# VainF/Diff-Pruning

Measured on NVIDIA H100. Metric: taylor_score_unet_fwd_bwd_passes_per_sec, higher is better.
Workload: dtype f32

## Files before the change

### diff-pruning_b200/csrc/conv_tc.cu

```cuda
#include <cuda.h>
#include <cuda_fp16.h>
#include "common.cuh"
#include "sm90.cuh"
#include "sm90_host.cuh"

namespace {
using namespace sm90;

constexpr int BM = 128, BK = 64;
constexpr int A_BYTES = BM * 32 * 4;

struct TcParams {
  int Nimg, H, W;
  int Nout;
  int kchunks;
  int bw, bh, bn, tiles_w, tiles_h;
  float* y; long long ldy;
  const float* bias;
  const float* rowadd; long long ld_rowadd;
  const float* residual; long long ld_res;
  int accumulate;
  int vec4;
  int ntaps;
  signed char dh[9], dw[9], wt[9];
  int os, oa, ob, Ho, Wo;
  int in_stride;
  float alpha;
  int b_from_img;
  const uint32_t* amax_a;
  const uint32_t* amax_b;
  uint32_t* amax_out;
  int ksplit, it_per_split;
  float* ws; long long ws_split_stride; int ws_ld;
  const float* gx; long long gldx;
  int gH, gW, gC, gQ, gPQ, gS, gstride, gpad_t, gpad_l, gM;
  int relu;
};

__device__ __forceinline__ int amax_exponent(const uint32_t* slot) {
  const int E = (int)((__ldg(slot) >> 23) & 0xFFu);
  return min(max(E, 14), 254);
}
__device__ __forceinline__ float scale_up(int E) { return __uint_as_float((uint32_t)(267 - E) << 23); }
__device__ __forceinline__ float scale_dn(int E) { return __uint_as_float((uint32_t)(E - 13) << 23); }
constexpr float LO_SCALE = 2048.f, LO_UNSCALE = 1.f / 2048.f;
__device__ __forceinline__ void split2(float a, float b, uint32_t& h, uint32_t& l) {
  const __half2 hh = __floats2half2_rn(a, b);
  const float2 hf = __half22float2(hh);
  const __half2 ll = __floats2half2_rn((a - hf.x) * LO_SCALE, (b - hf.y) * LO_SCALE);
  h = *reinterpret_cast<const uint32_t*>(&hh);
  l = *reinterpret_cast<const uint32_t*>(&ll);
}
__device__ __forceinline__ void split1(float v, __half& h, __half& l) {
  h = __float2half_rn(v);
  l = __float2half_rn((v - __half2float(h)) * LO_SCALE);
}

constexpr int PS_STAGES = 3, PS_BN = 128;
constexpr int PS_B_BYTES = PS_BN * BK * 2;
constexpr int PS_STAGE_BYTES = 2 * A_BYTES + 2 * PS_B_BYTES;

template <bool ANY>
__global__ void __launch_bounds__(THREADS, 1)
conv_tc_ps_kernel(const __grid_constant__ CUtensorMap mapA, const __grid_constant__ CUtensorMap mapBh,
                  const __grid_constant__ CUtensorMap mapBl, const TcParams p, const int tiles_m, const int total_tiles) {
  const int total_work = total_tiles * p.ksplit;
  extern __shared__ uint8_t smem_raw[];
  const uint32_t raw = smem_u32(smem_raw);
  const uint32_t pad_to = ((raw + 1023u) & ~1023u) - raw;
  uint8_t* smem = smem_raw + pad_to;
  const uint32_t sbase = raw + pad_to;
  const uint32_t bar0 = sbase + PS_STAGES * PS_STAGE_BYTES;
  auto full_bar = [&](int s) { return bar0 + 8u * s; };
  auto empty_bar = [&](int s) { return bar0 + 8u * (PS_STAGES + s); };
  const int wg = threadIdx.x >> 7, tid = threadIdx.x & 127;
  if (threadIdx.x == 0) {
    for (int s = 0; s < PS_STAGES; ++s) { mbar_init(full_bar(s), ANY ? 1 + 128 : 1); mbar_init(empty_bar(s), 8); }
    mbar_init_fence();
  }
  __syncthreads();
  const int iters_per_tile = p.ntaps * p.kchunks;

  auto tile_coords = [&](int tile, int& q0, int& p0, int& n0, int& nblk) {
    nblk = tile / tiles_m;
    const int tile_m = tile - nblk * tiles_m;
    const int tw = tile_m % p.tiles_w;
    const int th = (tile_m / p.tiles_w) % p.tiles_h;
    const int tn = tile_m / (p.tiles_w * p.tiles_h);
    q0 = tw * p.bw; p0 = th * p.bh; n0 = tn * p.bn;
  };

  if (wg == 0) {
    setmaxnreg_dec<40>();
    if constexpr (ANY) {
      const int t = threadIdx.x;
      if (t == 0) { prefetch_map(&mapBh); prefetch_map(&mapBl); }
      const uint32_t sw = (uint32_t)(t & 7);
      uint32_t g = 0;
      for (int wi = blockIdx.x; wi < total_work; wi += gridDim.x) {
        const int tile = wi % total_tiles, it0 = (wi / total_tiles) * p.it_per_split, it1 = min(iters_per_tile, it0 + p.it_per_split);
        const int nblk = tile / tiles_m, m = (tile - nblk * tiles_m) * BM + t;
        const bool mv = m < p.gM;
        const int n = mv ? m / p.gPQ : 0, rem = m - n * p.gPQ, pq = rem / p.gQ;
        const int hb = pq * p.gstride - p.gpad_t, wb = (rem - pq * p.gQ) * p.gstride - p.gpad_l;
        const float* xn = p.gx + (long long)n * p.gH * p.gW * p.gldx;
        for (int it = it0; it < it1; ++it, ++g) {
          const int s = g % PS_STAGES;
          const uint32_t ph = (g / PS_STAGES) & 1u;
          mbar_wait(empty_bar(s), ph ^ 1u);
          const int tap = it / p.kchunks, kc = it - tap * p.kchunks;
          const int r = tap / p.gS, h = hb + r, w = wb + (tap - r * p.gS);
          const uint32_t st = sbase + s * PS_STAGE_BYTES;
          if (t == 0) {
            mbar_expect_tx(full_bar(s), 2 * PS_B_BYTES);
            tma_load_3d(st + 2 * A_BYTES, &mapBh, full_bar(s), kc * BK, nblk * PS_BN, tap);
            tma_load_3d(st + 2 * A_BYTES + PS_B_BYTES, &mapBl, full_bar(s), kc * BK, nblk * PS_BN, tap);
          }
          const bool v = mv && h >= 0 && h < p.gH && w >= 0 && w < p.gW;
          const int cleft = v ? p.gC - kc * BK : 0;
          const float* src = v ? xn + ((long long)h * p.gW + w) * p.gldx + kc * BK : p.gx;
#pragma unroll
          for (int j = 0; j < 16; ++j) {
            const int nb = min(max(cleft - 4 * j, 0), 4) * 4;
            cp_async16(st + (j >> 3) * A_BYTES + t * 128 + ((((uint32_t)j & 7u) ^ sw) << 4), nb ? src + 4 * j : p.gx, (uint32_t)nb);
          }
          cp_async_mbar_arrive(full_bar(s));
        }
      }
      return;
    }
    if (threadIdx.x == 0) {
      prefetch_map(&mapA); prefetch_map(&mapBh); prefetch_map(&mapBl);
      uint32_t g = 0;
      for (int wi = blockIdx.x; wi < total_work; wi += gridDim.x) {
        const int tile = wi % total_tiles, it0 = (wi / total_tiles) * p.it_per_split, it1 = min(iters_per_tile, it0 + p.it_per_split);
        int q0, p0, n0, nblk;
        tile_coords(tile, q0, p0, n0, nblk);
        for (int it = it0; it < it1; ++it, ++g) {
          const int s = g % PS_STAGES;
          const uint32_t ph = (g / PS_STAGES) & 1u;
          mbar_wait(empty_bar(s), ph ^ 1u);
          mbar_expect_tx(full_bar(s), PS_STAGE_BYTES);
          const int tap = it / p.kchunks, kc = it - tap * p.kchunks;
          const uint32_t st = sbase + s * PS_STAGE_BYTES;
          const int aw = q0 * p.in_stride + p.dw[tap], ah = p0 * p.in_stride + p.dh[tap];
          tma_load_4d(st, &mapA, full_bar(s), kc * BK, aw, ah, n0);
          tma_load_4d(st + A_BYTES, &mapA, full_bar(s), kc * BK + 32, aw, ah, n0);
          const int tapb = p.b_from_img ? n0 : p.wt[tap];
          tma_load_3d(st + 2 * A_BYTES, &mapBh, full_bar(s), kc * BK, nblk * PS_BN, tapb);
          tma_load_3d(st + 2 * A_BYTES + PS_B_BYTES, &mapBl, full_bar(s), kc * BK, nblk * PS_BN, tapb);
        }
      }
    }
    return;
  }
  setmaxnreg_inc<232>();
  const int c = wg - 1;
  const int warp = tid >> 5, lane = tid & 31;
  const uint32_t frag_row = (uint32_t)(64 * c + 16 * warp + (lane >> 2)) * 128 + 8 * (lane & 1);
  const uint32_t fsw = (uint32_t)(lane >> 2), fj = (uint32_t)((lane & 3) >> 1);
  const float sa = scale_up(amax_exponent(p.amax_a));
  const float f1 = scale_dn(amax_exponent(p.amax_a)), f2 = scale_dn(amax_exponent(p.amax_b)) * p.alpha;
  auto fin = [&](float main, float corr) { return fmaf(corr, LO_UNSCALE, main) * f1 * f2; };
  float amax = 0.f;
  uint32_t g = 0;
  for (int wi = blockIdx.x; wi < total_work; wi += gridDim.x) {
    const int tile = wi % total_tiles, it0 = (wi / total_tiles) * p.it_per_split, it1 = min(iters_per_tile, it0 + p.it_per_split);
    float acc[64], cor[64];
    uint32_t fh[2][4], fl[2][4];
    int prev_s = 0;
    for (int it = it0; it < it1; ++it, ++g) {
      const int s = g % PS_STAGES;
      const uint32_t ph = (g / PS_STAGES) & 1u;
      mbar_wait(full_bar(s), ph);
      const uint8_t* stp = smem + s * PS_STAGE_BYTES + frag_row;
      const uint32_t bst = sbase + s * PS_STAGE_BYTES + 2 * A_BYTES;
#pragma unroll
      for (int k = 0; k < BK / 16; ++k) {
        uint32_t (&ah)[4] = fh[k & 1];
        uint32_t (&al)[4] = fl[k & 1];
        const uint8_t* a = stp + (k >> 1) * A_BYTES;
        const uint32_t pos = ((4u * (k & 1) + fj) ^ fsw) << 4;
        const float2 v0 = *reinterpret_cast<const float2*>(a + pos), v1 = *reinterpret_cast<const float2*>(a + 1024 + pos);
        const float2 v2 = *reinterpret_cast<const float2*>(a + (pos ^ 32u)), v3 = *reinterpret_cast<const float2*>(a + 1024 + (pos ^ 32u));
        split2(v0.x * sa, v0.y * sa, ah[0], al[0]);
        split2(v1.x * sa, v1.y * sa, ah[1], al[1]);
        split2(v2.x * sa, v2.y * sa, ah[2], al[2]);
        split2(v3.x * sa, v3.y * sa, ah[3], al[3]);
        const uint64_t b_hi = desc_k(bst + k * 32), b_lo = desc_k(bst + PS_B_BYTES + k * 32);
        const uint32_t first = (it > it0 || k > 0) ? 1u : 0u;
        wgmma_fence();
        wgmma_f16_n128_rs<0>(acc, ah, b_hi, first);
        wgmma_f16_n128_rs<0>(cor, ah, b_lo, first);
        wgmma_f16_n128_rs<0>(cor, al, b_hi, 1u);
        wgmma_commit();
        wgmma_wait<1>();
        if (k == 0 && it > it0 && lane == 0) mbar_arrive(empty_bar(prev_s));
      }
      prev_s = s;
    }
    wgmma_wait<0>();
    fence_regs(acc); fence_regs(cor);
    if (lane == 0) mbar_arrive(empty_bar(prev_s));

    int q0, p0, n0, nblk;
    tile_coords(tile, q0, p0, n0, nblk);
#pragma unroll
    for (int i = 0; i < 2; ++i) {
      const int row = 64 * c + 16 * warp + (lane >> 2) + 8 * i;
      const int cb = 2 * (lane & 3);
      if (p.ksplit > 1) {
        float* wrow = p.ws + (long long)(wi / total_tiles) * p.ws_split_stride + ((long long)(tile - nblk * tiles_m) * BM + row) * p.ws_ld + nblk * PS_BN;
#pragma unroll
        for (int j = 0; j < 16; ++j)
          *reinterpret_cast<float2*>(wrow + 8 * j + cb) =
              make_float2(fin(acc[4 * j + 2 * i], cor[4 * j + 2 * i]), fin(acc[4 * j + 2 * i + 1], cor[4 * j + 2 * i + 1]));
        continue;
      }
      const int w_l = row % p.bw, h_l = (row / p.bw) % p.bh, n_l = row / (p.bw * p.bh);
      const int img = n0 + n_l;
      if (img >= p.Nimg) continue;
      if constexpr (ANY) { if (q0 + w_l >= p.Wo) continue; }
      const long long m = ((long long)img * p.Ho + ((p0 + h_l) * p.os + p.oa)) * p.Wo + ((q0 + w_l) * p.os + p.ob);
      float* yrow = p.y + m * p.ldy;
      const float* rrow = p.residual ? p.residual + m * p.ld_res : nullptr;
      const float* arow2 = p.rowadd ? p.rowadd + (long long)img * p.ld_rowadd : nullptr;
#pragma unroll
      for (int j = 0; j < 16; ++j) {
        const int col = nblk * PS_BN + 8 * j + cb;
        float o[2] = {fin(acc[4 * j + 2 * i], cor[4 * j + 2 * i]), fin(acc[4 * j + 2 * i + 1], cor[4 * j + 2 * i + 1])};
        if (p.vec4 && col + 2 <= p.Nout) {
          if (p.bias) { const float2 t = __ldg(reinterpret_cast<const float2*>(p.bias + col)); o[0] += t.x; o[1] += t.y; }
          if (arow2) { const float2 t = __ldg(reinterpret_cast<const float2*>(arow2 + col)); o[0] += t.x; o[1] += t.y; }
          if (rrow) { const float2 t = __ldg(reinterpret_cast<const float2*>(rrow + col)); o[0] += t.x; o[1] += t.y; }
          float2* dst = reinterpret_cast<float2*>(yrow + col);
          if (p.accumulate) { const float2 t = *dst; o[0] += t.x; o[1] += t.y; }
          if constexpr (ANY) { if (p.relu) { o[0] = fmaxf(o[0], 0.f); o[1] = fmaxf(o[1], 0.f); } }
          *dst = make_float2(o[0], o[1]);
          amax = fmaxf(amax, fmaxf(fabsf(o[0]), fabsf(o[1])));
        } else {
#pragma unroll
          for (int e = 0; e < 2; ++e) {
            const int cc = col + e;
            if (cc < p.Nout) {
              float ov = o[e];
              if (p.bias) ov += __ldg(p.bias + cc);
              if (arow2) ov += __ldg(arow2 + cc);
              if (rrow) ov += __ldg(rrow + cc);
              if (p.accumulate) ov += yrow[cc];
              if constexpr (ANY) { if (p.relu) ov = fmaxf(ov, 0.f); }
              yrow[cc] = ov;
              amax = fmaxf(amax, fabsf(ov));
            }
          }
        }
      }
    }
  }
  if (p.amax_out && p.ksplit == 1) amax_commit(p.amax_out, amax);
}

__global__ void __launch_bounds__(256) splitk_epilogue_kernel(const TcParams p, const int tiles_m) {
  const int c4 = (p.Nout + 3) >> 2;
  const long long total = (long long)tiles_m * BM * c4;
  float amax = 0.f;
  for (long long i = blockIdx.x * 256ll + threadIdx.x; i < total; i += (long long)gridDim.x * 256) {
    const long long grow = i / c4;
    const int c = (int)(i - grow * c4) << 2;
    const int tile_m = (int)(grow / BM), row = (int)(grow - (long long)tile_m * BM);
    const int tw = tile_m % p.tiles_w, th = (tile_m / p.tiles_w) % p.tiles_h, tn = tile_m / (p.tiles_w * p.tiles_h);
    const int w_l = row % p.bw, h_l = (row / p.bw) % p.bh, n_l = row / (p.bw * p.bh);
    const int img = tn * p.bn + n_l;
    if (img >= p.Nimg) continue;
    const float* src = p.ws + grow * p.ws_ld + c;
    float4 acc = *reinterpret_cast<const float4*>(src);
    for (int ks = 1; ks < p.ksplit; ++ks) {
      const float4 t = *reinterpret_cast<const float4*>(src + ks * p.ws_split_stride);
      acc.x += t.x; acc.y += t.y; acc.z += t.z; acc.w += t.w;
    }
    float o[4] = {acc.x, acc.y, acc.z, acc.w};
    const long long m = ((long long)img * p.Ho + ((th * p.bh + h_l) * p.os + p.oa)) * p.Wo + ((tw * p.bw + w_l) * p.os + p.ob);
    float* yrow = p.y + m * p.ldy;
#pragma unroll
    for (int e = 0; e < 4; ++e) {
      const int cc = c + e;
      if (cc < p.Nout) {
        float v = o[e];
        if (p.bias) v += __ldg(p.bias + cc);
        if (p.rowadd) v += __ldg(p.rowadd + (long long)img * p.ld_rowadd + cc);
        if (p.residual) v += __ldg(p.residual + m * p.ld_res + cc);
        if (p.accumulate) v += yrow[cc];
        yrow[cc] = v;
        amax = fmaxf(amax, fabsf(v));
      }
    }
  }
  if (p.amax_out) amax_commit(p.amax_out, amax);
}

__global__ void __launch_bounds__(256) splitk_flat_epilogue_kernel(const TcParams p) {
  const int c4 = (p.Nout + 3) >> 2;
  const long long total = (long long)p.gM * c4;
  float amax = 0.f;
  for (long long i = blockIdx.x * 256ll + threadIdx.x; i < total; i += (long long)gridDim.x * 256) {
    const long long m = i / c4;
    const int c = (int)(i - m * c4) << 2;
    const float* src = p.ws + m * p.ws_ld + c;
    float4 acc = *reinterpret_cast<const float4*>(src);
    for (int ks = 1; ks < p.ksplit; ++ks) {
      const float4 t = *reinterpret_cast<const float4*>(src + ks * p.ws_split_stride);
      acc.x += t.x; acc.y += t.y; acc.z += t.z; acc.w += t.w;
    }
    const float o[4] = {acc.x, acc.y, acc.z, acc.w};
    float* yrow = p.y + m * p.ldy;
#pragma unroll
    for (int e = 0; e < 4; ++e) {
      const int cc = c + e;
      if (cc < p.Nout) {
        float v = o[e];
        if (p.bias) v += __ldg(p.bias + cc);
        if (p.residual) v += __ldg(p.residual + m * p.ld_res + cc);
        if (p.accumulate) v += yrow[cc];
        if (p.relu) v = fmaxf(v, 0.f);
        yrow[cc] = v;
        amax = fmaxf(amax, fabsf(v));
      }
    }
  }
  if (p.amax_out) amax_commit(p.amax_out, amax);
}

struct WgParams {
  int Nimg, H, W, C, K;
  int R, S, pad;
  int bw, bh, bn, tiles_w, tiles_h;
  int total_chunks, chunks_per_split;
  int c_tiles;
  float* ws;
  int in_stride;
  const uint32_t* amax_x; const uint32_t* amax_y;
  float* bias_ws;
};
constexpr int WG_KPIX = 64;
constexpr int WG_BLK = WG_KPIX * 128;
constexpr int WG_STAGES = 3, WG_STAGE_BYTES = 8 * WG_BLK;

__global__ void __launch_bounds__(THREADS, 1)
wgrad_tc_kernel(const __grid_constant__ CUtensorMap mapDy, const __grid_constant__ CUtensorMap mapX, const WgParams p) {
  extern __shared__ uint8_t smem_raw[];
  const uint32_t raw = smem_u32(smem_raw);
  const uint32_t pad_to = ((raw + 1023u) & ~1023u) - raw;
  uint8_t* smem = smem_raw + pad_to;
  const uint32_t sbase = raw + pad_to;
  const uint32_t bar0 = sbase + WG_STAGES * WG_STAGE_BYTES;
  auto full_bar = [&](int s) { return bar0 + 8u * s; };
  auto empty_bar = [&](int s) { return bar0 + 8u * (WG_STAGES + s); };
  const int wg = threadIdx.x >> 7, tid = threadIdx.x & 127;
  if (threadIdx.x == 0) {
    for (int s = 0; s < WG_STAGES; ++s) { mbar_init(full_bar(s), 1); mbar_init(empty_bar(s), 8); }
    mbar_init_fence();
  }
  __syncthreads();

  const int T = p.R * p.S;
  int tile = blockIdx.x;
  const int tap = tile % T; tile /= T;
  const int ct = tile % p.c_tiles;
  const int kt = tile / p.c_tiles;
  const int r = tap / p.S, sx = tap - r * p.S;
  const int chunk0 = blockIdx.y * p.chunks_per_split;
  const int chunk1 = min(p.total_chunks, chunk0 + p.chunks_per_split);
  const int num_iters = max(0, chunk1 - chunk0);
  const int dy_boxes = min(4, (p.K - kt * 128 + 31) >> 5), x_boxes = min(4, (p.C - ct * 128 + 31) >> 5);

  if (wg == 0) {
    setmaxnreg_dec<24>();
    if (threadIdx.x == 0) {
      prefetch_map(&mapDy); prefetch_map(&mapX);
      for (int it = 0; it < num_iters; ++it) {
        const int s = it % WG_STAGES;
        const uint32_t ph = (uint32_t)(it / WG_STAGES) & 1u;
        mbar_wait(empty_bar(s), ph ^ 1u);
        mbar_expect_tx(full_bar(s), (uint32_t)((dy_boxes + x_boxes) * WG_BLK));
        const int chunk = chunk0 + it;
        const int tw = chunk % p.tiles_w;
        const int th = (chunk / p.tiles_w) % p.tiles_h;
        const int tn = chunk / (p.tiles_w * p.tiles_h);
        const int q0 = tw * p.bw, p0 = th * p.bh, n0 = tn * p.bn;
        const uint32_t st = sbase + s * WG_STAGE_BYTES;
        const int xw = q0 * p.in_stride + sx - p.pad, xh = p0 * p.in_stride + r - p.pad;
#pragma unroll
        for (int b = 0; b < 4; ++b) {
          const uint32_t slot = (uint32_t)((b & 1) * 2 + (b >> 1));
          if (b < dy_boxes) tma_load_4d(st + slot * WG_BLK, &mapDy, full_bar(s), kt * 128 + b * 32, q0, p0, n0);
          if (b < x_boxes) tma_load_4d(st + (4 + slot) * WG_BLK, &mapX, full_bar(s), ct * 128 + b * 32, xw, xh, n0);
        }
      }
    }
    return;
  }
  setmaxnreg_inc<240>();
  const int c = wg - 1;
  const int warp = tid >> 5, lane = tid & 31;
  const int Ey = amax_exponent(p.amax_y), Ex = amax_exponent(p.amax_x);
  const float sy = scale_up(Ey), sxs = scale_up(Ex);
  const bool dy_valid = 2 * c + (warp >> 1) < dy_boxes;
  const uint32_t cb = (uint32_t)(16 * (warp & 1) + (lane >> 2)), pe = (uint32_t)(2 * (lane & 3));
  const uint32_t dy_off = (uint32_t)((warp >> 1) * 2 + c) * WG_BLK + pe * 128 + (((cb >> 2) ^ pe) << 4) + (cb & 3) * 4;
  const int xp = tid & 63, xh = tid >> 6;
  const bool x_valid = 2 * c + xh < x_boxes;
  const uint32_t xsw = (uint32_t)(xp & 7);
  float bsum[2] = {0.f, 0.f};
  float acc[64], cor[64];
  int prev_s = 0;
  auto stage = [&](uint32_t (&fah)[4][4], uint32_t (&fal)[4][4], const int it) {
    const int s = it % WG_STAGES;
    const uint32_t ph = (uint32_t)(it / WG_STAGES) & 1u;
    mbar_wait(full_bar(s), ph);
    uint8_t* stp = smem + s * WG_STAGE_BYTES;
    uint8_t* x0 = stp + 4 * WG_BLK + c * WG_BLK + xp * 128;
    uint8_t* x1 = x0 + 2 * WG_BLK;
    float4 xv[8];
    if (x_valid) {
      const uint8_t* src = xh ? x1 : x0;
#pragma unroll
      for (int j = 0; j < 8; ++j) xv[j] = *reinterpret_cast<const float4*>(src + ((j ^ xsw) << 4));
    }
    named_sync(1 + c, 128);
    if (x_valid) {
#pragma unroll
      for (int m = 0; m < 4; ++m) {
        const float4 u0 = xv[2 * m], u1 = xv[2 * m + 1];
        uint4 hq, lq;
        split2(u0.x * sxs, u0.y * sxs, hq.x, lq.x);
        split2(u0.z * sxs, u0.w * sxs, hq.y, lq.y);
        split2(u1.x * sxs, u1.y * sxs, hq.z, lq.z);
        split2(u1.z * sxs, u1.w * sxs, hq.w, lq.w);
        const uint32_t pos = (uint32_t)(((4 * xh + m) ^ xsw) << 4);
        *reinterpret_cast<uint4*>(x0 + pos) = hq;
        *reinterpret_cast<uint4*>(x1 + pos) = lq;
      }
    }
    fence_proxy_async();
    named_sync(3, 256);
    if (dy_valid) {
#pragma unroll
      for (int k = 0; k < WG_KPIX / 16; ++k)
#pragma unroll
        for (int q = 0; q < 4; ++q) {
          const uint8_t* d = stp + (16 * k + 8 * (q >> 1)) * 128;
          const float v0 = *reinterpret_cast<const float*>(d + (dy_off ^ (32u * (q & 1))));
          const float v1 = *reinterpret_cast<const float*>(d + (dy_off ^ (32u * (q & 1) + 144u)));
          bsum[q & 1] += v0 + v1;
          split2(v0 * sy, v1 * sy, fah[k][q], fal[k][q]);
        }
    } else {
#pragma unroll
      for (int k = 0; k < WG_KPIX / 16; ++k)
#pragma unroll
        for (int q = 0; q < 4; ++q) fah[k][q] = fal[k][q] = 0u;
    }
    const uint32_t st = sbase + s * WG_STAGE_BYTES;
    wgmma_fence();
#pragma unroll
    for (int k = 0; k < WG_KPIX / 16; ++k) {
      const uint64_t b_hi = desc_mn(st + 4 * WG_BLK + k * 2048, WG_BLK), b_lo = desc_mn(st + 6 * WG_BLK + k * 2048, WG_BLK);
      const uint32_t first = (it > 0 || k > 0) ? 1u : 0u;
      wgmma_f16_n128_rs<1>(acc, fah[k], b_hi, first);
      wgmma_f16_n128_rs<1>(cor, fah[k], b_lo, first);
      wgmma_f16_n128_rs<1>(cor, fal[k], b_hi, 1u);
    }
    wgmma_commit();
    wgmma_wait<1>();
    if (it > 0 && lane == 0) mbar_arrive(empty_bar(prev_s));
    prev_s = s;
  };
  uint32_t fah0[4][4], fal0[4][4], fah1[4][4], fal1[4][4];
  int it = 0;
  for (; it + 1 < num_iters; it += 2) {
    stage(fah0, fal0, it);
    stage(fah1, fal1, it + 1);
  }
  if (it < num_iters) stage(fah0, fal0, it);
  wgmma_wait<0>();
  fence_regs(acc); fence_regs(cor);
#pragma unroll
  for (int i = 0; i < 2; ++i) {
    bsum[i] += __shfl_xor_sync(0xffffffffu, bsum[i], 1);
    bsum[i] += __shfl_xor_sync(0xffffffffu, bsum[i], 2);
  }
  const float f1 = scale_dn(Ey), f2 = scale_dn(Ex);
  const long long TC_ = (long long)T * p.C;
#pragma unroll
  for (int i = 0; i < 2; ++i) {
    const int kout = kt * 128 + 64 * c + 16 * warp + (lane >> 2) + 8 * i;
    if (kout >= p.K) continue;
    if (p.bias_ws && tap == 0 && ct == 0 && (lane & 3) == 0) p.bias_ws[(long long)blockIdx.y * p.K + kout] = bsum[i];
    float* wrow = p.ws + ((long long)blockIdx.y * p.K + kout) * TC_ + (long long)tap * p.C;
#pragma unroll
    for (int j = 0; j < 16; ++j)
#pragma unroll
      for (int e = 0; e < 2; ++e) {
        const int col = ct * 128 + 8 * j + 2 * (lane & 3) + e;
        if (col < p.C) wrow[col] = num_iters ? fmaf(cor[4 * j + 2 * i + e], LO_UNSCALE, acc[4 * j + 2 * i + e]) * f1 * f2 : 0.f;
      }
  }
}

constexpr int PS_SMEM = PS_STAGES * PS_STAGE_BYTES + 2048;
constexpr int WG_SMEM = WG_STAGES * WG_STAGE_BYTES + 2048;

static int wrow(int c) { return c > 64 ? ((c + 63) & ~63) : ((c + 7) & ~7); }

int tc_init() {
  static const int ok = [] {
    const bool set = runtime().encode &&
        cudaFuncSetAttribute(conv_tc_ps_kernel<false>, cudaFuncAttributeMaxDynamicSharedMemorySize, PS_SMEM) == cudaSuccess &&
        cudaFuncSetAttribute(conv_tc_ps_kernel<true>, cudaFuncAttributeMaxDynamicSharedMemorySize, PS_SMEM) == cudaSuccess &&
        cudaFuncSetAttribute(wgrad_tc_kernel, cudaFuncAttributeMaxDynamicSharedMemorySize, WG_SMEM) == cudaSuccess;
    (void)cudaGetLastError();
    return set ? 1 : 0;
  }();
  return ok;
}

constexpr int PS_MAX_SPLIT_STAGES = 147;

static int pick_ksplit(int tiles, int iters, int& it_per_split) {
  it_per_split = iters;
  const int sms = runtime().num_sms;
  int ks = 1;
  if (tiles * 2 <= sms && iters >= 8) {
    ks = sms / tiles;
    if (ks > iters / 4) ks = iters / 4;
    if (ks > 16) ks = 16;
  }
  const int chain_ks = (iters + PS_MAX_SPLIT_STAGES - 1) / PS_MAX_SPLIT_STAGES;
  if (ks < chain_ks) ks = chain_ks;
  if (ks < 2) return 1;
  it_per_split = (iters + ks - 1) / ks;
  return (iters + it_per_split - 1) / it_per_split;
}

struct TcPlan { int bw, bh, bn, tiles_w, tiles_h, tiles_m, n_tiles, ksplit, it_per_split; long long ws_floats; };
int plan_tc(const ConvGemm& g, bool flat, bool split, TcPlan& pl) {
  if (!tc_init()) return DP_ERR_UNSUPPORTED;
  if (flat) { pl.bw = BM; pl.bh = 1; pl.bn = 1; }
  else if (!pick_box(BM, g.H, g.W, pl.bw, pl.bh, pl.bn)) return DP_ERR_UNSUPPORTED;
  pl.tiles_w = (g.W + pl.bw - 1) / pl.bw; pl.tiles_h = g.H / pl.bh;
  pl.tiles_m = pl.tiles_w * pl.tiles_h * ((g.N + pl.bn - 1) / pl.bn);
  pl.n_tiles = (g.Nout + PS_BN - 1) / PS_BN;
  const int iters = g.taps.n * ((g.Kg + BK - 1) / BK);
  pl.ksplit = 1; pl.it_per_split = iters;
  if (split) pl.ksplit = pick_ksplit(pl.tiles_m * pl.n_tiles, iters, pl.it_per_split);
  pl.ws_floats = pl.ksplit > 1 ? (long long)pl.ksplit * pl.tiles_m * BM * pl.n_tiles * PS_BN : 0;
  return DP_OK;
}

struct TcLaunch {
  const float* act; long long ld_act; const uint32_t* amax_a;
  const void* w_hi; const void* w_lo; const uint32_t* amax_b; int T; int ldb = -1;
  float* out; long long ld_out;
  const float* bias = nullptr; const float* rowadd = nullptr; long long ld_rowadd = 0; const float* residual = nullptr; long long ld_res = 0;
  int accumulate = 0;
  float* ws = nullptr;
  uint32_t* amax_out = nullptr;
  float alpha = 1.0f;
  int b_from_img = 0;
  const dp_conv_args* gather = nullptr;
};

TcLaunch conv_launch(const dp_conv_args* a, bool dgrad) {
  TcLaunch l{};
  l.act = (const float*)(dgrad ? a->y : a->x); l.ld_act = dgrad ? a->ldy : a->ldx; l.amax_a = dgrad ? a->amax_y : a->amax_x;
  l.w_hi = a->w_tc_hi; l.w_lo = a->w_tc_lo; l.amax_b = a->amax_w; l.T = a->R * a->S;
  l.out = (float*)(dgrad ? a->x : a->y); l.ld_out = dgrad ? a->ldx : a->ldy;
  if (!dgrad) { l.bias = a->bias; l.rowadd = a->rowadd; l.ld_rowadd = a->ld_rowadd; l.residual = a->residual; l.ld_res = a->ld_res; }
  l.accumulate = (a->flags & DP_CONV_ACCUMULATE) ? 1 : 0;
  l.ws = a->workspace; l.amax_out = a->amax_out;
  return l;
}

int launch_tc(const ConvGemm& g, const TcLaunch& l, cudaStream_t st) {
  const bool any = l.gather != nullptr, split = l.ws && !l.b_from_img;
  TcPlan pl;
  if (plan_tc(g, any, split, pl) != DP_OK) return DP_ERR_UNSUPPORTED;
  if (!l.w_hi || !l.w_lo || !l.amax_a || !l.amax_b) return DP_ERR_UNSUPPORTED;
  if (l.ld_act % 4 || ((uintptr_t)l.act & 15) || ((uintptr_t)l.w_hi & 15) || ((uintptr_t)l.w_lo & 15)) return DP_ERR_UNSUPPORTED;
  if (l.b_from_img && pl.bn != 1) return DP_ERR_UNSUPPORTED;
  CUtensorMap mA, mBh, mBl;
  if (!any) {
    const int s = g.in_stride;
    const cuuint64_t Hin = (cuuint64_t)g.H * s, Win = (cuuint64_t)g.W * s;
    cuuint64_t dims[4] = {(cuuint64_t)g.Kg, Win, Hin, (cuuint64_t)g.N};
    cuuint64_t str[3] = {(cuuint64_t)l.ld_act * 4, Win * l.ld_act * 4, Hin * Win * l.ld_act * 4};
    cuuint32_t box[4] = {32u, (cuuint32_t)(pl.bw * s), (cuuint32_t)(pl.bh * s), (cuuint32_t)pl.bn};
    if (box[1] > 256 || box[2] > 256) return DP_ERR_UNSUPPORTED;
    if (!encode_map(&mA, CU_TENSOR_MAP_DATA_TYPE_FLOAT32, l.act, 4, dims, str, box, s)) return DP_ERR_UNSUPPORTED;
  }
  {
    const cuuint64_t Kp = (cuuint64_t)(l.ldb < 0 ? wrow(g.Kg) : l.ldb);
    if (Kp % 8) return DP_ERR_UNSUPPORTED;
    cuuint64_t dims[3] = {Kp, (cuuint64_t)g.Nout, (cuuint64_t)l.T};
    cuuint64_t str[2] = {Kp * 2, (cuuint64_t)g.Nout * Kp * 2};
    cuuint32_t box[3] = {(cuuint32_t)BK, (cuuint32_t)PS_BN, 1};
    if (!encode_map(&mBh, CU_TENSOR_MAP_DATA_TYPE_FLOAT16, l.w_hi, 3, dims, str, box) ||
        !encode_map(&mBl, CU_TENSOR_MAP_DATA_TYPE_FLOAT16, l.w_lo, 3, dims, str, box)) return DP_ERR_UNSUPPORTED;
  }
  TcParams p{};
  p.Nimg = g.N; p.H = g.H; p.W = g.W; p.Nout = g.Nout;
  p.ntaps = g.taps.n;
  for (int i = 0; i < 9; ++i) { p.dh[i] = g.taps.dh[i]; p.dw[i] = g.taps.dw[i]; p.wt[i] = g.taps.wt[i]; }
  p.os = g.os; p.oa = g.oa; p.ob = g.ob; p.Ho = g.Ho; p.Wo = g.Wo;
  p.alpha = l.alpha; p.b_from_img = l.b_from_img; p.in_stride = g.in_stride; p.amax_a = l.amax_a; p.amax_b = l.amax_b; p.amax_out = l.amax_out;
  p.kchunks = (g.Kg + BK - 1) / BK;
  p.bw = pl.bw; p.bh = pl.bh; p.bn = pl.bn; p.tiles_w = pl.tiles_w; p.tiles_h = pl.tiles_h;
  p.y = l.out; p.ldy = l.ld_out; p.bias = l.bias; p.rowadd = l.rowadd; p.ld_rowadd = l.ld_rowadd; p.residual = l.residual; p.ld_res = l.ld_res;
  p.accumulate = l.accumulate;
  p.vec4 = (al16(l.out, l.ld_out) && al16(l.bias, 0) && al16(l.rowadd, l.ld_rowadd) && al16(l.residual, l.ld_res)) ? 1 : 0;
  p.ksplit = pl.ksplit; p.it_per_split = pl.it_per_split;
  if (split) { p.ws = l.ws; p.ws_ld = pl.n_tiles * PS_BN; p.ws_split_stride = (long long)pl.tiles_m * BM * p.ws_ld; }
  if (any) {
    const dp_conv_args* a = l.gather;
    p.gx = l.act; p.gldx = l.ld_act; p.gH = a->H; p.gW = a->W; p.gC = a->C; p.gQ = a->Q; p.gPQ = a->P * a->Q; p.gS = a->S;
    p.gstride = a->stride; p.gpad_t = a->pad_t; p.gpad_l = a->pad_l; p.gM = g.W; p.relu = (a->flags & DP_CONV_RELU) ? 1 : 0;
  }
  const int sms = runtime().num_sms, total = pl.tiles_m * pl.n_tiles, work = total * p.ksplit, ctas = work < sms ? work : sms;
  if (any) conv_tc_ps_kernel<true><<<ctas, THREADS, PS_SMEM, st>>>(mBh, mBh, mBl, p, pl.tiles_m, total);
  else conv_tc_ps_kernel<false><<<ctas, THREADS, PS_SMEM, st>>>(mA, mBh, mBl, p, pl.tiles_m, total);
  if (p.ksplit > 1) {
    const int rc = dp_check_launch();
    if (rc) return rc;
    const long long items = (any ? (long long)g.W : (long long)pl.tiles_m * BM) * ((g.Nout + 3) / 4);
    long long blocks = (items + 255) / 256;
    if (blocks > sms * 8) blocks = sms * 8;
    if (any) splitk_flat_epilogue_kernel<<<(int)blocks, 256, 0, st>>>(p);
    else splitk_epilogue_kernel<<<(int)blocks, 256, 0, st>>>(p, pl.tiles_m);
  }
  return dp_check_launch();
}

__global__ void pack_tc_kernel(const float* __restrict__ w, int K, int C, int RS, int Cp, int Kp, __half* __restrict__ kc_hi,
                               __half* __restrict__ kc_lo, __half* __restrict__ ck_hi, __half* __restrict__ ck_lo,
                               const uint32_t* __restrict__ amax) {
  const float sw = scale_up(amax_exponent(amax));
  const long long na = (long long)RS * K * Cp, nb = (long long)RS * C * Kp;
  const long long total = na > nb ? na : nb;
  for (long long i = blockIdx.x * (long long)blockDim.x + threadIdx.x; i < total; i += (long long)gridDim.x * blockDim.x) {
    if (i < na && kc_hi) {
      int c = (int)(i % Cp); long long t = i / Cp; int k = (int)(t % K), tap = (int)(t / K);
      split1(c < C ? w[((long long)k * C + c) * RS + tap] * sw : 0.f, kc_hi[i], kc_lo[i]);
    }
    if (i < nb && ck_hi) {
      int k = (int)(i % Kp); long long t = i / Kp; int c = (int)(t % C), tap = (int)(t / C);
      split1(k < K ? w[((long long)k * C + c) * RS + tap] * sw : 0.f, ck_hi[i], ck_lo[i]);
    }
  }
}
__global__ void split_h3_rows_kernel(const float* __restrict__ x, long long ld, long long bs, int rows, int cols, int pitch, int vec,
                                     __half* __restrict__ hi, __half* __restrict__ lo, const uint32_t* __restrict__ amax) {
  const float sx = scale_up(amax_exponent(amax));
  const int groups = pitch >> 3;
  const long long total = (long long)rows * groups;
  const float* xb = x + (long long)blockIdx.y * bs;
  __half* hb = hi + (long long)blockIdx.y * rows * pitch;
  __half* lb = lo + (long long)blockIdx.y * rows * pitch;
  for (long long i = blockIdx.x * 256ll + threadIdx.x; i < total; i += (long long)gridDim.x * 256) {
    const long long r = i / groups;
    const int c0 = (int)(i - r * groups) << 3;
    const float* src = xb + r * ld + c0;
    float v[8];
    if (vec && c0 + 8 <= cols) {
      const float4 a = __ldg(reinterpret_cast<const float4*>(src)), b = __ldg(reinterpret_cast<const float4*>(src + 4));
      v[0] = a.x; v[1] = a.y; v[2] = a.z; v[3] = a.w; v[4] = b.x; v[5] = b.y; v[6] = b.z; v[7] = b.w;
    } else {
#pragma unroll
      for (int j = 0; j < 8; ++j) v[j] = (c0 + j < cols) ? __ldg(src + j) : 0.f;
    }
    uint4 h, l;
    split2(v[0] * sx, v[1] * sx, h.x, l.x); split2(v[2] * sx, v[3] * sx, h.y, l.y);
    split2(v[4] * sx, v[5] * sx, h.z, l.z); split2(v[6] * sx, v[7] * sx, h.w, l.w);
    *reinterpret_cast<uint4*>(hb + r * pitch + c0) = h;
    *reinterpret_cast<uint4*>(lb + r * pitch + c0) = l;
  }
}
__global__ void __launch_bounds__(256) split_h3_t_kernel(const float* __restrict__ x, long long ld, long long bs, int rows, int cols, int vec,
                                                         __half* __restrict__ hi, __half* __restrict__ lo, const uint32_t* __restrict__ amax) {
  __shared__ float t[64][65];
  const float sx = scale_up(amax_exponent(amax));
  const int b = blockIdx.z, r0 = blockIdx.y * 64, c0 = blockIdx.x * 64, tid = threadIdx.x;
  const float* xb = x + (long long)b * bs;
  {
    const int cc = (tid & 15) * 4, c = c0 + cc;
#pragma unroll
    for (int i = 0; i < 4; ++i) {
      const int rr = (tid >> 4) + 16 * i, r = r0 + rr;
      float4 v = make_float4(0.f, 0.f, 0.f, 0.f);
      if (r < rows) {
        const float* src = xb + (long long)r * ld + c;
        if (vec && c + 4 <= cols) v = __ldg(reinterpret_cast<const float4*>(src));
        else {
          if (c < cols) v.x = __ldg(src);
          if (c + 1 < cols) v.y = __ldg(src + 1);
          if (c + 2 < cols) v.z = __ldg(src + 2);
          if (c + 3 < cols) v.w = __ldg(src + 3);
        }
      }
      t[rr][cc] = v.x * sx; t[rr][cc + 1] = v.y * sx; t[rr][cc + 2] = v.z * sx; t[rr][cc + 3] = v.w * sx;
    }
  }
  __syncthreads();
  const int rows8 = (rows + 7) & ~7;
  const int c = c0 + (tid >> 2), rs = (tid & 3) * 16;
  if (c < cols) {
    const long long o = ((long long)b * cols + c) * rows8 + r0 + rs;
#pragma unroll
    for (int h8 = 0; h8 < 2; ++h8) {
      if (r0 + rs + 8 * h8 + 8 <= rows8) {
        uint4 h, l;
        const int rb = rs + 8 * h8, cl = tid >> 2;
        split2(t[rb][cl], t[rb + 1][cl], h.x, l.x); split2(t[rb + 2][cl], t[rb + 3][cl], h.y, l.y);
        split2(t[rb + 4][cl], t[rb + 5][cl], h.z, l.z); split2(t[rb + 6][cl], t[rb + 7][cl], h.w, l.w);
        *reinterpret_cast<uint4*>(hi + o + 8 * h8) = h;
        *reinterpret_cast<uint4*>(lo + o + 8 * h8) = l;
      }
    }
  }
}
__global__ void __launch_bounds__(256) transpose_batched_kernel(const float* __restrict__ in, float* __restrict__ out, int rows, int cols, int vec) {
  __shared__ float t[64][65];
  const int b = blockIdx.z, r0 = blockIdx.y * 64, c0 = blockIdx.x * 64, tid = threadIdx.x;
  const float* ib = in + (long long)b * rows * cols;
  float* ob = out + (long long)b * rows * cols;
  const int q4 = (tid & 15) * 4, l16 = tid >> 4;
#pragma unroll
  for (int i = 0; i < 4; ++i) {
    const int rr = l16 + 16 * i, r = r0 + rr, c = c0 + q4;
    float4 v = make_float4(0.f, 0.f, 0.f, 0.f);
    if (r < rows) {
      const float* src = ib + (long long)r * cols + c;
      if (vec && c + 4 <= cols) v = __ldg(reinterpret_cast<const float4*>(src));
      else {
        if (c < cols) v.x = __ldg(src);
        if (c + 1 < cols) v.y = __ldg(src + 1);
        if (c + 2 < cols) v.z = __ldg(src + 2);
        if (c + 3 < cols) v.w = __ldg(src + 3);
      }
    }
    t[rr][q4] = v.x; t[rr][q4 + 1] = v.y; t[rr][q4 + 2] = v.z; t[rr][q4 + 3] = v.w;
  }
  __syncthreads();
#pragma unroll
  for (int i = 0; i < 4; ++i) {
    const int cc = l16 + 16 * i, c = c0 + cc, r = r0 + q4;
    if (c < cols) {
      float* dst = ob + (long long)c * rows + r;
      if (vec && r + 4 <= rows) *reinterpret_cast<float4*>(dst) = make_float4(t[q4][cc], t[q4 + 1][cc], t[q4 + 2][cc], t[q4 + 3][cc]);
      else {
        if (r < rows) dst[0] = t[q4][cc];
        if (r + 1 < rows) dst[1] = t[q4 + 1][cc];
        if (r + 2 < rows) dst[2] = t[q4 + 2][cc];
        if (r + 3 < rows) dst[3] = t[q4 + 3][cc];
      }
    }
  }
}
}

extern "C" int dp_split_h3(const float* x, int64_t ld, int64_t bs, int32_t batch, int32_t rows, int32_t cols, int32_t transpose,
                           const uint32_t* amax, void* hi, void* lo, dp_stream_t stream) {
  DP_REQUIRE(x && hi && lo && amax, DP_ERR_NULL);
  DP_REQUIRE(batch > 0 && rows > 0 && cols > 0 && ld >= cols && batch <= 65535, DP_ERR_SHAPE);
  if (!transpose) {
    const int pitch = (cols + 7) & ~7;
    const int vec = ((((uintptr_t)x) & 15) == 0 && ld % 4 == 0 && bs % 4 == 0) ? 1 : 0;
    long long blocks = ((long long)rows * (pitch >> 3) + 255) / 256;
    if (blocks > runtime().num_sms * 8) blocks = runtime().num_sms * 8;
    split_h3_rows_kernel<<<dim3((unsigned)blocks, (unsigned)batch), 256, 0, (cudaStream_t)stream>>>(x, ld, bs, rows, cols, pitch, vec, (__half*)hi,
                                                                                                (__half*)lo, amax);
  } else {
    const int vec = ((((uintptr_t)x) & 15) == 0 && ld % 4 == 0 && bs % 4 == 0) ? 1 : 0;
    DP_REQUIRE((((uintptr_t)hi) & 15) == 0 && (((uintptr_t)lo) & 15) == 0, DP_ERR_ALIGN);
    dim3 grid((cols + 63) / 64, (((rows + 7) & ~7) + 63) / 64, batch);
    split_h3_t_kernel<<<grid, 256, 0, (cudaStream_t)stream>>>(x, ld, bs, rows, cols, vec, (__half*)hi, (__half*)lo, amax);
  }
  return dp_check_launch();
}
extern "C" int dp_transpose_batched(const float* in, float* out, int32_t batch, int32_t rows, int32_t cols, dp_stream_t stream) {
  DP_REQUIRE(in && out, DP_ERR_NULL);
  DP_REQUIRE(batch > 0 && rows > 0 && cols > 0 && batch <= 65535, DP_ERR_SHAPE);
  const int vec = ((((uintptr_t)in) & 15) == 0 && (((uintptr_t)out) & 15) == 0 && rows % 4 == 0 && cols % 4 == 0) ? 1 : 0;
  dim3 grid((cols + 63) / 64, (rows + 63) / 64, batch);
  transpose_batched_kernel<<<grid, 256, 0, (cudaStream_t)stream>>>(in, out, rows, cols, vec);
  return dp_check_launch();
}
extern "C" int dp_gemm_nt_tc(const dp_gemm_nt_args* a, dp_stream_t stream) {
  DP_REQUIRE(a && a->A && a->b_hi && a->b_lo && a->C, DP_ERR_NULL);
  DP_REQUIRE(a->batch > 0 && a->H > 0 && a->W > 0 && a->Kg > 0 && a->N > 0 && a->ld_a >= a->Kg && a->ldc >= a->N, DP_ERR_SHAPE);
  const ConvGemm g = {TapTable{1}, a->batch, a->H, a->W, a->Kg, a->N, 1, 0, 0, a->H, a->W, 1};
  return launch_tc(g, {.act = a->A, .ld_act = a->ld_a, .amax_a = a->amax_a, .w_hi = a->b_hi, .w_lo = a->b_lo, .amax_b = a->amax_b,
                       .T = a->batch, .ldb = (a->Kg + 7) & ~7, .out = a->C, .ld_out = a->ldc, .amax_out = a->amax_out, .alpha = a->alpha,
                       .b_from_img = 1},
                   (cudaStream_t)stream);
}

int dp_tc_runtime_ok() { return tc_init(); }

int dp_conv2d_fprop_tc(const dp_conv_args* a, dp_stream_t stream) {
  if (!a || !a->x || !a->y) return DP_ERR_UNSUPPORTED;
  if (a->flags & DP_CONV_RELU) return DP_ERR_UNSUPPORTED;
  if (!box_geometry(a)) return DP_ERR_UNSUPPORTED;
  if (a->N <= 0 || a->H <= 0 || a->W <= 0 || a->C <= 0 || a->K <= 0 || a->ldx < a->C || a->ldy < a->K) return DP_ERR_UNSUPPORTED;
  ConvGemm g[4];
  conv_gemms(a, 0, g);
  return launch_tc(g[0], conv_launch(a, false), (cudaStream_t)stream);
}

constexpr int ANY_MIN_C = 32;
int any_gemm(const dp_conv_args* a, ConvGemm& g) {
  if (a->N <= 0 || a->H <= 0 || a->W <= 0 || a->C <= 0 || a->K <= 0 || a->P <= 0 || a->Q <= 0 || a->R <= 0 || a->S <= 0) return DP_ERR_UNSUPPORTED;
  if (a->C < ANY_MIN_C || (a->stride != 1 && a->stride != 2) || a->pad_t < 0 || a->pad_l < 0 || a->rowadd) return DP_ERR_UNSUPPORTED;
  if ((long long)a->N * a->P * a->Q >= (1ll << 31) || (long long)a->R * a->S > 65535) return DP_ERR_UNSUPPORTED;
  const int M = a->N * a->P * a->Q;
  g = {TapTable{a->R * a->S}, 1, 1, M, a->C, a->K, 1, 0, 0, 1, M, 1};
  return DP_OK;
}
int dp_conv2d_fprop_tc_any(const dp_conv_args* a, dp_stream_t stream) {
  ConvGemm g;
  if (!a || any_gemm(a, g) != DP_OK || !a->x || !a->y) return DP_ERR_UNSUPPORTED;
  TcLaunch l = conv_launch(a, false);
  l.gather = a;
  return launch_tc(g, l, (cudaStream_t)stream);
}

int dp_conv2d_dgrad_tc(const dp_conv_args* a, dp_stream_t stream) {
  if (!a || !a->x || !a->y) return DP_ERR_UNSUPPORTED;
  if (a->N <= 0 || a->H <= 0 || a->W <= 0 || a->C <= 0 || a->K <= 0 || a->ldx < a->C || a->ldy < a->K) return DP_ERR_UNSUPPORTED;
  if (a->stride == 1 ? !box_geometry(a) : !(a->stride == 2 && a->R == 3 && a->S == 3 && a->H == 2 * a->P && a->W == 2 * a->Q))
    return DP_ERR_UNSUPPORTED;
  ConvGemm g[4];
  const int n = conv_gemms(a, 1, g);
  const TcLaunch l = conv_launch(a, true);
  for (int c = 0; c < n; ++c) {
    const int rc = launch_tc(g[c], l, (cudaStream_t)stream);
    if (rc != DP_OK) return (c == 0 || rc != DP_ERR_UNSUPPORTED) ? rc : DP_ERR_SHAPE;
  }
  return DP_OK;
}

extern "C" long long dp_conv_splitk_workspace_floats(const dp_conv_args* a, int op) {
  TcPlan pl;
  if (a && op == 0 && (a->flags & DP_CONV_ANY_GEOMETRY)) {
    dp_conv_args b = *a;
    b.flags &= ~DP_CONV_ANY_GEOMETRY;
    long long need = (a->flags & DP_CONV_RELU) ? 0 : dp_conv_splitk_workspace_floats(&b, 0);
    ConvGemm g;
    if (any_gemm(a, g) == DP_OK && plan_tc(g, true, true, pl) == DP_OK && pl.ws_floats > need) need = pl.ws_floats;
    return need;
  }
  if (!a || a->N <= 0 || a->H <= 0 || a->W <= 0 || a->C <= 0 || a->K <= 0 || a->R != a->S || (a->R != 1 && a->R != 3)) return 0;
  long long need = 0;
  ConvGemm g[4];
  for (int c = 0, n = conv_gemms(a, op, g); c < n; ++c)
    if (plan_tc(g[c], false, true, pl) == DP_OK && pl.ws_floats > need) need = pl.ws_floats;
  return need;
}

int dp_conv2d_wgrad_tc(const dp_conv_args* a, dp_stream_t stream) {
  if (!a || !a->x || !a->y || !a->workspace) return DP_ERR_UNSUPPORTED;
  if (!tc_init()) return DP_ERR_UNSUPPORTED;
  if (!box_geometry(a) || a->splits < 1) return DP_ERR_UNSUPPORTED;
  if (a->ldx % 4 || a->ldy % 4 || ((uintptr_t)a->x & 15) || ((uintptr_t)a->y & 15)) return DP_ERR_UNSUPPORTED;
  int bw, bh, bn;
  if (!a->amax_x || !a->amax_y) return DP_ERR_UNSUPPORTED;
  if (!pick_box(WG_KPIX, a->P, a->Q, bw, bh, bn)) return DP_ERR_UNSUPPORTED;
  const int img_boxes = (a->N + bn - 1) / bn;
  CUtensorMap mDy, mX;
  {
    cuuint64_t dims[4] = {(cuuint64_t)a->K, (cuuint64_t)a->Q, (cuuint64_t)a->P, (cuuint64_t)a->N};
    cuuint64_t str[3] = {(cuuint64_t)a->ldy * 4, (cuuint64_t)a->Q * a->ldy * 4, (cuuint64_t)a->P * a->Q * a->ldy * 4};
    cuuint32_t box[4] = {32, (cuuint32_t)bw, (cuuint32_t)bh, (cuuint32_t)bn};
    if (!encode_map(&mDy, CU_TENSOR_MAP_DATA_TYPE_FLOAT32, a->y, 4, dims, str, box)) return DP_ERR_UNSUPPORTED;
  }
  {
    cuuint64_t dims[4] = {(cuuint64_t)a->C, (cuuint64_t)a->W, (cuuint64_t)a->H, (cuuint64_t)a->N};
    cuuint64_t str[3] = {(cuuint64_t)a->ldx * 4, (cuuint64_t)a->W * a->ldx * 4, (cuuint64_t)a->H * a->W * a->ldx * 4};
    cuuint32_t box[4] = {32, (cuuint32_t)(bw * a->stride), (cuuint32_t)(bh * a->stride), (cuuint32_t)bn};
    if (box[1] > 256 || box[2] > 256) return DP_ERR_UNSUPPORTED;
    if (!encode_map(&mX, CU_TENSOR_MAP_DATA_TYPE_FLOAT32, a->x, 4, dims, str, box, a->stride)) return DP_ERR_UNSUPPORTED;
  }
  WgParams p{};
  p.Nimg = a->N; p.H = a->P; p.W = a->Q; p.C = a->C; p.K = a->K; p.R = a->R; p.S = a->S; p.pad = a->pad_t; p.in_stride = a->stride;
  p.bw = bw; p.bh = bh; p.bn = bn; p.tiles_w = a->Q / bw; p.tiles_h = a->P / bh;
  p.total_chunks = p.tiles_w * p.tiles_h * img_boxes;
  p.amax_x = a->amax_x; p.amax_y = a->amax_y; p.bias_ws = a->bias_ws;
  p.chunks_per_split = (p.total_chunks + a->splits - 1) / a->splits;
  p.c_tiles = (a->C + 127) / 128;
  p.ws = a->workspace;
  const int k_tiles = (a->K + 127) / 128;
  dim3 grid((unsigned)(k_tiles * p.c_tiles * a->R * a->S), (unsigned)a->splits);
  wgrad_tc_kernel<<<grid, THREADS, WG_SMEM, (cudaStream_t)stream>>>(mDy, mX, p);
  return dp_check_launch();
}

extern "C" int dp_pack_conv_weight_tc(const float* w, int32_t K, int32_t C, int32_t R, int32_t S, void* kc_hi, void* kc_lo,
                                      void* ck_hi, void* ck_lo, uint32_t* amax_w, dp_stream_t stream) {
  DP_REQUIRE(w && amax_w, DP_ERR_NULL);
  DP_REQUIRE((kc_hi == nullptr) == (kc_lo == nullptr) && (ck_hi == nullptr) == (ck_lo == nullptr), DP_ERR_NULL);
  DP_REQUIRE(K > 0 && C > 0 && R > 0 && S > 0, DP_ERR_SHAPE);
  if (cudaMemsetAsync(amax_w, 0, sizeof(uint32_t), (cudaStream_t)stream) != cudaSuccess) return dp_check_launch();
  int rc = dp_amax(w, (int64_t)C * R * S, K, C * R * S, amax_w, stream);
  if (rc) return rc;
  const int Cp = wrow(C), Kp = wrow(K);
  long long total = (long long)R * S * ((long long)K * Cp > (long long)C * Kp ? (long long)K * Cp : (long long)C * Kp);
  int blocks = (int)((total + 255) / 256);
  if (blocks > runtime().num_sms * 16) blocks = runtime().num_sms * 16;
  pack_tc_kernel<<<blocks, 256, 0, (cudaStream_t)stream>>>(w, K, C, R * S, Cp, Kp, (__half*)kc_hi, (__half*)kc_lo, (__half*)ck_hi, (__half*)ck_lo,
                                                           amax_w);
  return dp_check_launch();
}

extern "C" int dp_tc_weight_row(int channels) { return channels > 0 ? wrow(channels) : 0; }
```

Measured before the change: 23.57.

## Load halo activation tile once per k-chunk and reuse it across 3x3 taps

Adds a HALO variant of the implicit-GEMM conv kernel for dense stride-1 3x3 convolutions without split-K. A (bw+2)x(bh+2) activation halo box is TMA-loaded once per k-chunk into double-buffered shared memory, and the nine taps read shifted windows of it, in place of reloading the A tile for every tap. Weight stages shrink to B only and the iteration order changes to kchunk-major with taps inner. This cuts global/L2 activation traffic roughly ninefold, at the cost of more shared memory, extra barriers and more complex swizzle addressing.

```diff
diff --git a/diff-pruning_b200/csrc/conv_tc.cu b/diff-pruning_b200/csrc/conv_tc.cu
--- a/diff-pruning_b200/csrc/conv_tc.cu
+++ b/diff-pruning_b200/csrc/conv_tc.cu
@@ -60,7 +60,10 @@
 constexpr int PS_B_BYTES = PS_BN * BK * 2;
 constexpr int PS_STAGE_BYTES = 2 * A_BYTES + 2 * PS_B_BYTES;
 
-template <bool ANY>
+__host__ __device__ constexpr int ps_halo_box(int bw, int bh, int bn) { return ((bw + 2) * (bh + 2) * bn * 128 + 1023) & ~1023; }
+constexpr int PS_HALO_B_STAGE = 2 * PS_B_BYTES;
+
+template <bool ANY, bool HALO = false>
 __global__ void __launch_bounds__(THREADS, 1)
 conv_tc_ps_kernel(const __grid_constant__ CUtensorMap mapA, const __grid_constant__ CUtensorMap mapBh,
                   const __grid_constant__ CUtensorMap mapBl, const TcParams p, const int tiles_m, const int total_tiles) {
@@ -70,12 +73,18 @@
   const uint32_t pad_to = ((raw + 1023u) & ~1023u) - raw;
   uint8_t* smem = smem_raw + pad_to;
   const uint32_t sbase = raw + pad_to;
-  const uint32_t bar0 = sbase + PS_STAGES * PS_STAGE_BYTES;
+  constexpr int B_STAGE = HALO ? PS_HALO_B_STAGE : PS_STAGE_BYTES, B_OFF = HALO ? 0 : 2 * A_BYTES;
+  const uint32_t hbox = HALO ? (uint32_t)ps_halo_box(p.bw, p.bh, p.bn) : 0u;
+  const uint32_t hbase = sbase + PS_STAGES * B_STAGE;
+  const uint32_t bar0 = HALO ? hbase + 4 * hbox : sbase + PS_STAGES * PS_STAGE_BYTES;
   auto full_bar = [&](int s) { return bar0 + 8u * s; };
   auto empty_bar = [&](int s) { return bar0 + 8u * (PS_STAGES + s); };
+  auto halo_full = [&](int b) { return bar0 + 8u * (2 * PS_STAGES + b); };
+  auto halo_empty = [&](int b) { return bar0 + 8u * (2 * PS_STAGES + 2 + b); };
   const int wg = threadIdx.x >> 7, tid = threadIdx.x & 127;
   if (threadIdx.x == 0) {
     for (int s = 0; s < PS_STAGES; ++s) { mbar_init(full_bar(s), ANY ? 1 + 128 : 1); mbar_init(empty_bar(s), 8); }
+    if constexpr (HALO) for (int b = 0; b < 2; ++b) { mbar_init(halo_full(b), 1); mbar_init(halo_empty(b), 8); }
     mbar_init_fence();
   }
   __syncthreads();
@@ -129,6 +138,44 @@
       }
       return;
     }
+    if constexpr (HALO) {
+      if (threadIdx.x == 0) {
+        prefetch_map(&mapA); prefetch_map(&mapBh); prefetch_map(&mapBl);
+        const uint32_t hbytes = (uint32_t)((p.bw + 2) * (p.bh + 2) * p.bn) * 128u;
+        int hwi = blockIdx.x, hkc = 0;
+        uint32_t hq = 0;
+        auto load_halo = [&] {
+          if (hwi >= total_work) return;
+          const int b = hq & 1;
+          mbar_wait(halo_empty(b), ((hq >> 1) & 1u) ^ 1u);
+          mbar_expect_tx(halo_full(b), 2 * hbytes);
+          int q0, p0, n0, nblk;
+          tile_coords(hwi, q0, p0, n0, nblk);
+          const uint32_t dst = hbase + 2 * hbox * b;
+          tma_load_4d(dst, &mapA, halo_full(b), hkc * BK, q0 - 1, p0 - 1, n0);
+          tma_load_4d(dst + hbox, &mapA, halo_full(b), hkc * BK + 32, q0 - 1, p0 - 1, n0);
+          ++hq;
+          if (++hkc == p.kchunks) { hkc = 0; hwi += gridDim.x; }
+        };
+        load_halo();
+        uint32_t g = 0;
+        for (int wi = blockIdx.x; wi < total_work; wi += gridDim.x) {
+          const int nblk = wi / tiles_m;
+          for (int kc = 0; kc < p.kchunks; ++kc)
+            for (int tap = 0; tap < 9; ++tap, ++g) {
+              const int s = g % PS_STAGES;
+              const uint32_t ph = (g / PS_STAGES) & 1u;
+              mbar_wait(empty_bar(s), ph ^ 1u);
+              mbar_expect_tx(full_bar(s), 2 * PS_B_BYTES);
+              const uint32_t st = sbase + s * B_STAGE;
+              tma_load_3d(st, &mapBh, full_bar(s), kc * BK, nblk * PS_BN, p.wt[tap]);
+              tma_load_3d(st + PS_B_BYTES, &mapBl, full_bar(s), kc * BK, nblk * PS_BN, p.wt[tap]);
+              if (tap == 2) load_halo();
+            }
+        }
+      }
+      return;
+    }
     if (threadIdx.x == 0) {
       prefetch_map(&mapA); prefetch_map(&mapBh); prefetch_map(&mapBl);
       uint32_t g = 0;
@@ -162,6 +209,17 @@
   const float sa = scale_up(amax_exponent(p.amax_a));
   const float f1 = scale_dn(amax_exponent(p.amax_a)), f2 = scale_dn(amax_exponent(p.amax_b)) * p.alpha;
   auto fin = [&](float main, float corr) { return fmaf(corr, LO_UNSCALE, main) * f1 * f2; };
+  int hp0 = 0, hp1 = 0;
+  if constexpr (HALO) {
+    auto hpix = [&](int row) {
+      const int w_l = row % p.bw, h_l = (row / p.bw) % p.bh, n_l = row / (p.bw * p.bh);
+      return (n_l * (p.bh + 2) + h_l) * (p.bw + 2) + w_l;
+    };
+    hp0 = hpix(64 * c + 16 * warp + (lane >> 2));
+    hp1 = hpix(64 * c + 16 * warp + (lane >> 2) + 8);
+  }
+  uint32_t hq = 0;
+  int tap = 0;
   float amax = 0.f;
   uint32_t g = 0;
   for (int wi = blockIdx.x; wi < total_work; wi += gridDim.x) {
@@ -174,15 +232,32 @@
       const uint32_t ph = (g / PS_STAGES) & 1u;
       mbar_wait(full_bar(s), ph);
       const uint8_t* stp = smem + s * PS_STAGE_BYTES + frag_row;
-      const uint32_t bst = sbase + s * PS_STAGE_BYTES + 2 * A_BYTES;
+      const uint32_t bst = sbase + s * B_STAGE + B_OFF;
+      const uint8_t *h0 = nullptr, *h1 = nullptr;
+      uint32_t hs0 = 0, hs1 = 0;
+      if constexpr (HALO) {
+        if (tap == 0) mbar_wait(halo_full(hq & 1), (hq >> 1) & 1u);
+        const int r = tap / 3, x0 = hp0 + r * (p.bw + 2) + (tap - 3 * r), x1 = x0 + (hp1 - hp0);
+        const uint8_t* hb = smem + (hbase - sbase) + 2 * hbox * (hq & 1) + 8 * (lane & 1);
+        h0 = hb + x0 * 128; h1 = hb + x1 * 128;
+        hs0 = (uint32_t)x0 & 7u; hs1 = (uint32_t)x1 & 7u;
+      }
 #pragma unroll
       for (int k = 0; k < BK / 16; ++k) {
         uint32_t (&ah)[4] = fh[k & 1];
         uint32_t (&al)[4] = fl[k & 1];
-        const uint8_t* a = stp + (k >> 1) * A_BYTES;
-        const uint32_t pos = ((4u * (k & 1) + fj) ^ fsw) << 4;
-        const float2 v0 = *reinterpret_cast<const float2*>(a + pos), v1 = *reinterpret_cast<const float2*>(a + 1024 + pos);
-        const float2 v2 = *reinterpret_cast<const float2*>(a + (pos ^ 32u)), v3 = *reinterpret_cast<const float2*>(a + 1024 + (pos ^ 32u));
+        float2 v0, v1, v2, v3;
+        if constexpr (HALO) {
+          const uint8_t *a0 = h0 + (k >> 1) * hbox, *a1 = h1 + (k >> 1) * hbox;
+          const uint32_t pos0 = ((4u * (k & 1) + fj) ^ hs0) << 4, pos1 = ((4u * (k & 1) + fj) ^ hs1) << 4;
+          v0 = *reinterpret_cast<const float2*>(a0 + pos0); v1 = *reinterpret_cast<const float2*>(a1 + pos1);
+          v2 = *reinterpret_cast<const float2*>(a0 + (pos0 ^ 32u)); v3 = *reinterpret_cast<const float2*>(a1 + (pos1 ^ 32u));
+        } else {
+          const uint8_t* a = stp + (k >> 1) * A_BYTES;
+          const uint32_t pos = ((4u * (k & 1) + fj) ^ fsw) << 4;
+          v0 = *reinterpret_cast<const float2*>(a + pos); v1 = *reinterpret_cast<const float2*>(a + 1024 + pos);
+          v2 = *reinterpret_cast<const float2*>(a + (pos ^ 32u)); v3 = *reinterpret_cast<const float2*>(a + 1024 + (pos ^ 32u));
+        }
         split2(v0.x * sa, v0.y * sa, ah[0], al[0]);
         split2(v1.x * sa, v1.y * sa, ah[1], al[1]);
         split2(v2.x * sa, v2.y * sa, ah[2], al[2]);
@@ -195,12 +270,15 @@
         wgmma_f16_n128_rs<0>(cor, al, b_hi, 1u);
         wgmma_commit();
         wgmma_wait<1>();
+        if constexpr (HALO) { if (k == 0 && it > it0 && tap == 0 && lane == 0) mbar_arrive(halo_empty((hq - 1) & 1)); }
         if (k == 0 && it > it0 && lane == 0) mbar_arrive(empty_bar(prev_s));
       }
       prev_s = s;
+      if constexpr (HALO) { if (++tap == 9) { tap = 0; ++hq; } }
     }
     wgmma_wait<0>();
     fence_regs(acc); fence_regs(cor);
+    if constexpr (HALO) { if (lane == 0) mbar_arrive(halo_empty((hq - 1) & 1)); }
     if (lane == 0) mbar_arrive(empty_bar(prev_s));
 
     int q0, p0, n0, nblk;
@@ -509,6 +587,8 @@
 
 constexpr int PS_SMEM = PS_STAGES * PS_STAGE_BYTES + 2048;
 constexpr int WG_SMEM = WG_STAGES * WG_STAGE_BYTES + 2048;
+constexpr int PS_HALO_SMEM_MAX = 227 * 1024;
+static int ps_halo_smem(int bw, int bh, int bn) { return PS_STAGES * PS_HALO_B_STAGE + 4 * ps_halo_box(bw, bh, bn) + 2048; }
 
 static int wrow(int c) { return c > 64 ? ((c + 63) & ~63) : ((c + 7) & ~7); }
 
@@ -517,6 +597,7 @@
     const bool set = runtime().encode &&
         cudaFuncSetAttribute(conv_tc_ps_kernel<false>, cudaFuncAttributeMaxDynamicSharedMemorySize, PS_SMEM) == cudaSuccess &&
         cudaFuncSetAttribute(conv_tc_ps_kernel<true>, cudaFuncAttributeMaxDynamicSharedMemorySize, PS_SMEM) == cudaSuccess &&
+        cudaFuncSetAttribute(conv_tc_ps_kernel<false, true>, cudaFuncAttributeMaxDynamicSharedMemorySize, PS_HALO_SMEM_MAX) == cudaSuccess &&
         cudaFuncSetAttribute(wgrad_tc_kernel, cudaFuncAttributeMaxDynamicSharedMemorySize, WG_SMEM) == cudaSuccess;
     (void)cudaGetLastError();
     return set ? 1 : 0;
@@ -542,7 +623,13 @@
   return (iters + it_per_split - 1) / it_per_split;
 }
 
-struct TcPlan { int bw, bh, bn, tiles_w, tiles_h, tiles_m, n_tiles, ksplit, it_per_split; long long ws_floats; };
+struct TcPlan { int bw, bh, bn, tiles_w, tiles_h, tiles_m, n_tiles, ksplit, it_per_split; long long ws_floats; bool halo; };
+static bool dense_3x3(const TapTable& t) {
+  if (t.n != 9) return false;
+  for (int i = 0; i < 9; ++i)
+    if (t.dh[i] != i / 3 - 1 || t.dw[i] != i % 3 - 1) return false;
+  return true;
+}
 int plan_tc(const ConvGemm& g, bool flat, bool split, TcPlan& pl) {
   if (!tc_init()) return DP_ERR_UNSUPPORTED;
   if (flat) { pl.bw = BM; pl.bh = 1; pl.bn = 1; }
@@ -554,6 +641,8 @@
   pl.ksplit = 1; pl.it_per_split = iters;
   if (split) pl.ksplit = pick_ksplit(pl.tiles_m * pl.n_tiles, iters, pl.it_per_split);
   pl.ws_floats = pl.ksplit > 1 ? (long long)pl.ksplit * pl.tiles_m * BM * pl.n_tiles * PS_BN : 0;
+  pl.halo = !flat && pl.ksplit == 1 && g.in_stride == 1 && dense_3x3(g.taps) && pl.bn == 1 && pl.bw >= 8 && pl.bw % 8 == 0 &&
+            ps_halo_smem(pl.bw, pl.bh, pl.bn) <= PS_HALO_SMEM_MAX;
   return DP_OK;
 }
 
@@ -588,6 +677,7 @@
   if (!l.w_hi || !l.w_lo || !l.amax_a || !l.amax_b) return DP_ERR_UNSUPPORTED;
   if (l.ld_act % 4 || ((uintptr_t)l.act & 15) || ((uintptr_t)l.w_hi & 15) || ((uintptr_t)l.w_lo & 15)) return DP_ERR_UNSUPPORTED;
   if (l.b_from_img && pl.bn != 1) return DP_ERR_UNSUPPORTED;
+  const bool halo = pl.halo && !l.b_from_img;
   CUtensorMap mA, mBh, mBl;
   if (!any) {
     const int s = g.in_stride;
@@ -595,6 +685,7 @@
     cuuint64_t dims[4] = {(cuuint64_t)g.Kg, Win, Hin, (cuuint64_t)g.N};
     cuuint64_t str[3] = {(cuuint64_t)l.ld_act * 4, Win * l.ld_act * 4, Hin * Win * l.ld_act * 4};
     cuuint32_t box[4] = {32u, (cuuint32_t)(pl.bw * s), (cuuint32_t)(pl.bh * s), (cuuint32_t)pl.bn};
+    if (halo) { box[1] = (cuuint32_t)(pl.bw + 2); box[2] = (cuuint32_t)(pl.bh + 2); }
     if (box[1] > 256 || box[2] > 256) return DP_ERR_UNSUPPORTED;
     if (!encode_map(&mA, CU_TENSOR_MAP_DATA_TYPE_FLOAT32, l.act, 4, dims, str, box, s)) return DP_ERR_UNSUPPORTED;
   }
@@ -627,6 +718,7 @@
   }
   const int sms = runtime().num_sms, total = pl.tiles_m * pl.n_tiles, work = total * p.ksplit, ctas = work < sms ? work : sms;
   if (any) conv_tc_ps_kernel<true><<<ctas, THREADS, PS_SMEM, st>>>(mBh, mBh, mBl, p, pl.tiles_m, total);
+  else if (halo) conv_tc_ps_kernel<false, true><<<ctas, THREADS, ps_halo_smem(pl.bw, pl.bh, pl.bn), st>>>(mA, mBh, mBl, p, pl.tiles_m, total);
   else conv_tc_ps_kernel<false><<<ctas, THREADS, PS_SMEM, st>>>(mA, mBh, mBl, p, pl.tiles_m, total);
   if (p.ksplit > 1) {
     const int rc = dp_check_launch();
```

Measured after the change: 23.75, median of 6. Within noise of the previous version (+0.7%).
